# Cibiv/NextGenMap

Measured on AMD Instinct MI355X. Metric: mapped reads/sec + SW Gcells/sec, 150bp vs GRCh38, at 1/2/4/8 MI355X, higher is better.
Workload: dtype int32

## Files before the change

### include/ngm_pipeline.h

```cpp
#ifndef NGM_PIPELINE_H
#define NGM_PIPELINE_H

#include <stddef.h>
#include <stdint.h>

#ifdef __cplusplus
extern "C" {
#endif

typedef struct ngm_ref ngm_ref;
typedef struct ngm_mapper ngm_mapper;

typedef struct ngm_ref_params {
	int kmer;
	int kmer_skip;
	int bin_size;
} ngm_ref_params;

const char *ngm_pipeline_last_error(void);

ngm_ref *ngm_ref_create(int device, const ngm_ref_params *p, int n_contigs, const char *const *names,
		const uint8_t *const *seqs, const uint64_t *lens);
ngm_ref *ngm_ref_create_from_fasta(int device, const ngm_ref_params *p, const char *path);
ngm_ref *ngm_ref_create_from_cache(int device, const ngm_ref_params *params, const char *fasta_path);
// ... 127 lines not shown
int ngm_mapper_set_reference_cs_batch(ngm_mapper *m, int reads);

int ngm_mapper_path_counters(ngm_mapper *m, uint64_t out[8]);

int ngm_mapper_order_table_reads(ngm_mapper *m, uint64_t *out);

int ngm_debug_pair_walk(uint32_t cnt_a, int len_a, uint32_t cnt_b, int len_b, const uint32_t *loc, const uint32_t *sv, const float *score, const uint32_t *rank,
		float cutoff, int min_insert, int max_insert, uint32_t *out_a, uint32_t *out_b, int *mq_a, int *mq_b, uint64_t cap, float *combo_score, int *combo_dist, int *combo_a, int *combo_b,
		uint64_t *n_combo);

int ngm_debug_pair_eval(uint64_t n, const float *pair_score, const int *dist, const int *ia, const int *ib, int avg, int out_all[6], int out_kept[6]);

int ngm_debug_select_top1(int device, int n_reads, const uint32_t *base, const uint32_t *count, uint64_t n_cand, const float *scores, const uint32_t *loc,
		const uint32_t *strand_votes, uint32_t *winner, int32_t *mapq, int32_t *n_best, float *best_score);

int ngm_mapper_heavy_counters(ngm_mapper *m, uint64_t out[4]);

int ngm_mapper_cs_counters(ngm_mapper *m, uint64_t out[3]);

typedef struct ngm_stats_comm ngm_stats_comm;
int ngm_stats_unique_id(char hex[257]);
ngm_stats_comm *ngm_stats_comm_create(int device, int rank, int world, const char *hex);
int ngm_stats_allreduce(ngm_stats_comm *c, int64_t v[8]);
void ngm_stats_comm_destroy(ngm_stats_comm *c);
int ngm_mapper_last_pair_stats(ngm_mapper *m, uint64_t out[3]);

int ngm_mapper_last_kernel_ms(ngm_mapper *m, float ms[8]);
float ngm_mapper_last_order_replay_ms(ngm_mapper *m);

int ngm_mapper_set_argos(ngm_mapper *m, float min_score);
// ... 12 lines not shown
```

### nextgenmap_amd/csrc/cigar_device.h

```cpp
#pragma once

#include <hip/hip_runtime.h>
#include <stdint.h>

#include "sw_device.h"

namespace ngm {

struct CigarDevOut {
	uint32_t cig_off, md_off;
	uint16_t cig_len, md_len;
	int32_t position_offset, qstart, qend, nm;
	float identity, score_token;
	int32_t flags;
};

__device__ __forceinline__ uint32_t packed_class(const uint32_t *base, int m_base, int j) {
	const uint32_t w = base[(size_t) (m_base + (j >> 3)) * kSlots];
	const int b = j & 7;
	return (b < 4) ? (w >> (8 * b)) & 15u : (w >> (8 * (b - 4) + 4)) & 15u;
}
__device__ __forceinline__ char class_to_char(uint32_t c) {
	switch (c) { case 0: return 'A'; case 1: return 'C'; case 2: return 'G'; case 3: return 'T'; case 4: return 'x'; case 5: return 'N'; default: return 0; }
}
// ... 134 lines not shown
	__syncthreads();
	const unsigned long long base = s_base;
	if (!live) return;
	if (need) {
		if (base + total > capacity) o.flags &= ~1;
		else {
			const unsigned long long off = base + before;
			o.cig_off = (uint32_t) off; o.md_off = (uint32_t) off + o.cig_len;
			for (int t = 0; t < co; ++t) bytes[off + t] = cg[t];
			for (int t = 0; t < mo; ++t) bytes[off + co + t] = mdp[t];
		}
	}
	out[j] = o;
}

}
```

### nextgenmap_amd/csrc/engine_internal.h

```cpp
#pragma once

#include <algorithm>

#include <hip/hip_runtime.h>

#include <cstdint>
#include <string>

#include "../../include/ngm_hip.h"
#include "sw_device.h"
#include "affine_device.h"
#include "jit.h"

namespace ngm {
template <typename T>
struct DevBuf {
	T *p = nullptr;
	size_t cap = 0;
	int reserve(size_t n) {
		if (n <= cap) return 0;
		if (p) (void) hipFree(p);
		p = nullptr;
		cap = 0;
		const size_t want = n + std::min<size_t>(n / 8, ((size_t) 64 << 20) / sizeof(T));
		if (hipMalloc(&p, want * sizeof(T)) == hipSuccess) { cap = want; return 0; }
		if (hipMalloc(&p, n * sizeof(T)) != hipSuccess) return -1;
// ... 35 lines not shown
	ngm::DevBuf<uint32_t> packed;
	ngm::DevBuf<uint16_t> lens, blk_rows;
	ngm::DevBuf<uint8_t> d_ref, d_qry, d_pair_dir;
	const uint8_t *pair_dir = nullptr;
	ngm::DevBuf<float> d_scores;
	ngm::DevBuf<uint32_t> dirs;
	ngm::DevBuf<int32_t> d_records;
	ngm::DevBuf<uint16_t> d_runs;
	ngm::PinnedBuf<uint8_t> h_ref, h_qry;
	ngm::PinnedBuf<float> h_scores;
	ngm::PinnedBuf<int32_t> h_records;
	ngm::PinnedBuf<uint16_t> h_runs;
	bool profiling = false;
	hipEvent_t ev[4] = {nullptr, nullptr, nullptr, nullptr};
	bool ev_valid[3] = {false, false, false};
	std::string error;
};

namespace ngm {
int engine_reserve(ngm_hip_ctx *ctx, int n);
int engine_score_packed(ngm_hip_ctx *ctx, int mode, int n, float *d_scores, hipStream_t st);
int engine_align_packed(ngm_hip_ctx *ctx, int mode, int n, int32_t *d_records, uint16_t *d_runs, int run_stride, hipStream_t st);
}
```

### nextgenmap_amd/csrc/gather_device.h

```cpp
#pragma once

#include <hip/hip_runtime.h>
#include <stdint.h>

#include "sw_device.h"

namespace ngm {

struct WindowGeom {
	uint64_t concat_len;
	int buffer_len;
	int half_corridor;
};

__device__ __forceinline__ uint32_t window_class(const uint32_t *__restrict__ genome, const WindowGeom &G, uint64_t offset, int j) {
	uint64_t len = (uint64_t) G.buffer_len - 2;
	if (offset >= G.concat_len) return 5u;
	uint64_t end = 0;
	if (offset + len > G.concat_len) { end = offset + len - G.concat_len; len -= end; }
	const uint64_t emitted = ((offset & 1) ? 1 : 0) + 2 * ((len + 1) / 2);
	const uint64_t jj = (uint64_t) j;
	if (jj < emitted) {
		if ((len & 1) && jj == emitted - 1) return 4u;
		const uint64_t pos = offset + jj;
// ... 206 lines not shown
		if (small) { const uint32_t at = bs + (uint32_t) __popcll(ms & below); list_small[at] = (uint32_t) pi; info[pi] = -2 - (int32_t) at; }
		if (large) { const uint32_t at = bl + (uint32_t) __popcll(ml & below); list_large[at] = (uint32_t) pi; info[pi] = -2 - (int32_t) (at + (1u << 30)); }
		if (choice) return;
	}
	if (!live) return;
	if (ca != 1u || cb != 1u) { info[pi] = -1; return; }
	const uint32_t ba = cand_base[ra], bb = cand_base[rb];
	const uint64_t l1 = pair_loc[ba], l2 = pair_loc[bb];
	const int cur = (int) ((l2 > l1) ? l2 - l1 + (uint64_t) read_len[rb] : l1 - l2 + (uint64_t) read_len[ra]);
	const float ps = scores[ba] + scores[bb];
	const bool found = cur > min_d && cur < max_d && ps > 0.0f;
	if (found) { mapq[ra] = 60; mapq[rb] = 60; n_best[ra] = 0; n_best[rb] = 0; }
	info[pi] = found ? ((cur << 1) | 1) : 0;
}

__global__ void expand_pairs_kernel(int n_reads, const uint32_t *__restrict__ cand_base, const uint32_t *__restrict__ cand_count,
		uint32_t *__restrict__ pair_read) {
	const int r = blockIdx.x;
	const uint32_t b = cand_base[r], n = cand_count[r];
	for (uint32_t j = threadIdx.x; j < n; j += blockDim.x) pair_read[b + j] = (uint32_t) r;
}

__global__ void collect_winners_kernel(int n_reads, const uint32_t *__restrict__ winner, const uint32_t *__restrict__ pair_loc,
		const uint32_t *__restrict__ pair_sv, const uint32_t *__restrict__ slot_of_read, uint32_t *__restrict__ a_read,
		uint32_t *__restrict__ a_loc, uint32_t *__restrict__ a_sv) {
	const int r = blockIdx.x * blockDim.x + threadIdx.x;
	if (r >= n_reads) return;
	const uint32_t w = winner[r];
	if (w == 0xFFFFFFFFu) return;
	const uint32_t s = slot_of_read[r];
	a_read[s] = (uint32_t) r;
	a_loc[s] = pair_loc[w];
	a_sv[s] = pair_sv[w];
}

// ... 14 lines not shown
```

### nextgenmap_amd/csrc/mapper.cpp

```cpp
#define NGM_SAM_KERNELS
#include "mapper_internal.h"
#include <rocprim/rocprim.hpp>
#include "align_device.h"
#include "gather_device.h"

using ngm::DevGuard;
using ngm::GpuStage;
using ngm::run_cs;
using ngm::cs_host_arrays;
using ngm::candidate_order;
using ngm::candidate_order_wait;

namespace ngm {
StageLock g_stage_lock[16][2];
std::atomic<long long> g_stage_hold_us[3], g_stage_wait_us[3];
}
using ngm::g_stage_hold_us;
using ngm::g_stage_wait_us;

namespace {

int upload_reads(ngm_mapper *m, int n, const char *reads) {
	const size_t bytes = (size_t) n * m->prm.qry_max_len;
	if (m->d_reads.reserve(bytes)) { ngm::pipeline_set_error("out of device memory (reads)"); return -12; }
// ... 24 lines not shown
		char ch;
		if (jj < emitted) ch = ((len & 1) && jj == emitted - 1) ? 'x' : class_char(r->host_cls[offset + jj]);
		else if (jj < emitted + end) ch = 'x';
		else ch = 0;
		out[j] = ch;
	}
}

}

namespace ngm {
int score_candidates(ngm_mapper *m, int n, uint64_t np, int alt_dir) {
	const ngm_ref *r = m->ref;
	ngm_hip_ctx *eng = m->eng;
	const int q = m->prm.qry_max_len, c = m->prm.corridor;
	hipLaunchKernelGGL(ngm::expand_pairs_kernel, dim3(n), dim3(64), 0, m->st, n, m->d_cand_base.p, m->d_cand_count.p, m->d_pair_read.p);
	const int nb = (int) ((np + ngm::kSlots - 1) / ngm::kSlots);
	ngm::WindowGeom Gs{r->n_bases - 1, ((q + c) | 1) + 1, c >> 1};
	hipLaunchKernelGGL(ngm::gather_pairs_kernel, dim3(nb), dim3(256), 0, m->st, m->d_reads.p, m->d_read_len.p, q, r->d_genome, Gs,
			m->d_pair_read.p, m->d_out_loc.p, m->d_out_sv.p, (int) np, eng->RW, eng->FW, eng->packed.p, eng->lens.p, eng->blk_rows.p, alt_dir);
	MAP_HIP_TRY(hipGetLastError());
	MAP_HIP_TRY(hipEventRecord(m->ev[2], m->st));
	if (int rc = ngm::engine_score_packed(eng, m->prm.mode, (int) np, m->d_scores.p, m->st)) { ngm::pipeline_set_error("%s", ngm_hip_last_error(eng)); return rc; }
	MAP_HIP_TRY(hipEventRecord(m->ev[3], m->st));
	return 0;
}
}

extern "C" {

int ngm_ref_decode(const ngm_ref *r, uint64_t offset, int buffer_len, char *out) {
// ... 955 lines not shown
		if (m->d_a_read.reserve(na) || m->d_a_loc.reserve(na) || m->d_a_sv.reserve(na) || m->d_records.reserve((size_t) na * 8) ||
				m->d_runs.reserve((size_t) na * rs)) { ngm::pipeline_set_error("out of device memory (align stage)"); return -12; }
		if (int rc = ngm::engine_reserve(eng, na)) { ngm::pipeline_set_error("%s", ngm_hip_last_error(eng)); return rc; }
		MAP_HIP_TRY(hipMemcpyAsync(m->d_a_read.p, a_read.data(), (size_t) na * 4, hipMemcpyHostToDevice, m->st));
		MAP_HIP_TRY(hipMemcpyAsync(m->d_a_loc.p, a_loc.data(), (size_t) na * 4, hipMemcpyHostToDevice, m->st));
		MAP_HIP_TRY(hipMemcpyAsync(m->d_a_sv.p, a_sv.data(), (size_t) na * 4, hipMemcpyHostToDevice, m->st));
		MAP_HIP_TRY(hipStreamSynchronize(m->st));
		stage_align.acquire();
		MAP_HIP_TRY(hipEventRecord(m->ev[5], m->st));
		ngm::WindowGeom Ga{r->n_bases - 1, align_buf_len, c >> 1};
		hipLaunchKernelGGL(ngm::gather_pairs_kernel, dim3((na + ngm::kSlots - 1) / ngm::kSlots), dim3(256), 0, m->st, m->d_reads.p, m->d_read_len.p, q,
				r->d_genome, Ga, m->d_a_read.p, m->d_a_loc.p, m->d_a_sv.p, na, eng->RW, eng->FW, eng->packed.p, eng->lens.p, eng->blk_rows.p, alt_dir);
		MAP_HIP_TRY(hipGetLastError());
		MAP_HIP_TRY(hipEventRecord(m->ev[6], m->st));
		const bool was_prof = eng->profiling;
		eng->profiling = true;
		if (int rc = ngm::engine_align_packed(eng, mode, na, m->d_records.p, m->d_runs.p, rs, m->st)) { eng->profiling = was_prof; ngm::pipeline_set_error("%s", ngm_hip_last_error(eng)); return rc; }
		eng->profiling = was_prof;
		MAP_HIP_TRY(hipEventRecord(m->ev[7], m->st));
		if (m->d_runs_c.reserve((size_t) na * rs)) { ngm::pipeline_set_error("out of device memory (runs)"); return -12; }
		MAP_HIP_TRY(hipMemsetAsync(m->d_total.p, 0, 8, m->st));
		hipLaunchKernelGGL(ngm::compact_runs_kernel, dim3((na + 255) / 256), dim3(256), 0, m->st, na, m->d_records.p, m->d_runs.p, rs,
				m->d_runs_c.p, m->d_total.p);
		MAP_HIP_TRY(hipGetLastError());
		unsigned long long n_runs_total = 0, n_str_total = 0;
		if (!dev_strings) { MAP_HIP_TRY(hipEventRecord(m->ev[8], m->st)); }
		if (dev_strings) {
			const unsigned long long scap = (unsigned long long) na * 96ull + 4096ull;
			if (m->d_cigout.reserve(na) || m->d_str.reserve(scap) || m->p_cigout.reserve(na)) { ngm::pipeline_set_error("out of memory (CIGAR strings)"); return -12; }
			MAP_HIP_TRY(hipMemsetAsync(m->d_total.p + 8, 0, 8, m->st));
			const bool affine = m->prm.personality == NGM_PERSONALITY_AFFINE;
			if (affine) hipLaunchKernelGGL(ngm::cigar_strings_kernel<true>, dim3((na + 255) / 256), dim3(256), 0, m->st, na, m->d_records.p, m->d_runs_c.p, eng->packed.p, eng->RW, eng->FW,
					m->d_read_len.p, m->d_a_read.p, m->prm.variant == NGM_VARIANT_OCL_CPU ? 1 : 0, m->prm.hard_clip, m->prm.silent_clip, m->d_cigout.p, m->d_str.p, scap,
					(unsigned long long *) (m->d_total.p + 8), 0);
			else hipLaunchKernelGGL(ngm::cigar_strings_kernel<false>, dim3((na + 255) / 256), dim3(256), 0, m->st, na, m->d_records.p, m->d_runs_c.p, eng->packed.p, eng->RW, eng->FW,
					m->d_read_len.p, m->d_a_read.p, m->prm.variant == NGM_VARIANT_OCL_CPU ? 1 : 0, m->prm.hard_clip, m->prm.silent_clip, m->d_cigout.p, m->d_str.p, scap,
					(unsigned long long *) (m->d_total.p + 8), alt_cigar);
			MAP_HIP_TRY(hipGetLastError());
			MAP_HIP_TRY(hipEventRecord(m->ev[8], m->st));
			MAP_HIP_TRY(hipMemcpyAsync(m->p_cigout.p, m->d_cigout.p, (size_t) na * sizeof(ngm::CigarDevOut), hipMemcpyDeviceToHost, m->st));
			MAP_HIP_TRY(hipMemcpyAsync(&n_str_total, m->d_total.p + 8, 8, hipMemcpyDeviceToHost, m->st));
		}
		MAP_HIP_TRY(hipMemcpyAsync(h_rec, m->d_records.p, (size_t) na * 8 * 4, hipMemcpyDeviceToHost, m->st));
		MAP_HIP_TRY(hipMemcpyAsync(&n_runs_total, m->d_total.p, 8, hipMemcpyDeviceToHost, m->st));
		stage_align.done_after(m->ev[8]);
		MAP_HIP_TRY(hipStreamSynchronize(m->st));
		if (m->p_runs.reserve(n_runs_total + 1)) { ngm::pipeline_set_error("out of pinned host memory"); return -12; }
		h_runs = m->p_runs.p;
		MAP_HIP_TRY(hipMemcpy(h_runs, m->d_runs_c.p, n_runs_total * 2, hipMemcpyDeviceToHost));
		if (dev_strings) {
			n_str_total = std::min<unsigned long long>(n_str_total, (unsigned long long) na * 96ull + 4096ull);
			str_base = n_str_total;
			if (m->p_str.reserve(n_str_total + 1)) { ngm::pipeline_set_error("out of pinned host memory"); return -12; }
			if (n_str_total && !sam) MAP_HIP_TRY(hipMemcpy(m->p_str.p, m->d_str.p, n_str_total, hipMemcpyDeviceToHost));
		}
	}
	stage_align.done();

	lap(3);
	ngm::SamRef *sam_refs = sam ? m->p_sam_refs.p : nullptr;
	std::mutex extra_mu;
	std::vector<char> extra;
	parallel_for(n, [&](int lo, int hi) {
		for (int i = lo; i < hi; ++i) for (int t = 0; t < topn; ++t) {
			const size_t o = (size_t) i * topn + t;
			ngm_hit &h = hits[o];
			memset(&h, 0, sizeof(h));
			h.n_candidates = (int) m->h_count[i];
			h.max_votes = m->h_maxv[i];
// ... 298 lines not shown
		MAP_HIP_TRY(hipMemcpy(d_sc.p, scores, (size_t) n_cand * 4, hipMemcpyHostToDevice));
		MAP_HIP_TRY(hipMemcpy(d_loc.p, loc, (size_t) n_cand * 4, hipMemcpyHostToDevice));
		MAP_HIP_TRY(hipMemcpy(d_sv.p, strand_votes, (size_t) n_cand * 4, hipMemcpyHostToDevice));
	}
	hipLaunchKernelGGL(ngm::select_top1_kernel, dim3((n_reads + 255) / 256), dim3(256), 0, 0, n_reads, d_base.p, d_count.p, d_sc.p, d_loc.p, d_sv.p, d_win.p, d_mq.p, d_nb.p, d_best.p);
	MAP_HIP_TRY(hipGetLastError());
	MAP_HIP_TRY(hipDeviceSynchronize());
	MAP_HIP_TRY(hipMemcpy(winner, d_win.p, (size_t) n_reads * 4, hipMemcpyDeviceToHost));
	MAP_HIP_TRY(hipMemcpy(mapq, d_mq.p, (size_t) n_reads * 4, hipMemcpyDeviceToHost));
	MAP_HIP_TRY(hipMemcpy(n_best, d_nb.p, (size_t) n_reads * 4, hipMemcpyDeviceToHost));
	MAP_HIP_TRY(hipMemcpy(best_score, d_best.p, (size_t) n_reads * 4, hipMemcpyDeviceToHost));
	d_base.release(); d_count.release(); d_loc.release(); d_sv.release(); d_win.release(); d_mq.release(); d_nb.release(); d_sc.release(); d_best.release();
	return 0;
}

int ngm_mapper_heavy_counters(ngm_mapper *m, uint64_t out[4]) {
	if (!m || !out) return -22;
	out[0] = m->st_heavy_second; out[1] = m->st_heavy_restart; out[2] = m->st_heavy_sent_on; out[3] = m->st_pool_regrown;
	return 0;
}

int ngm_mapper_order_table_reads(ngm_mapper *m, uint64_t *out) {
	if (!m || !out) return -22;
	*out = m->st_order_table;
	return 0;
}

int ngm_mapper_cs_counters(ngm_mapper *m, uint64_t out[3]) {
	if (!m) return -22;
	out[0] = m->cs_kmers; out[1] = m->cs_hits; out[2] = m->n_cand;
// ... 19 lines not shown
```

### nextgenmap_amd/csrc/ngm_hip.cpp

```cpp
#include "../../include/ngm_hip.h"

#include <hip/hip_runtime.h>

#include <algorithm>

#include <cstdarg>
#include <cstdio>
#include <cstdlib>
#include <cstring>
#include <mutex>
#include <string>
#include <vector>

#define NGM_ENGINE_KERNELS
#include "engine_internal.h"
#include "align_device.h"
#include "affine_device.h"
#include "cigar_md.h"
#include "jit.h"

namespace {

thread_local std::string g_last_error;

// ... 139 lines not shown
	const bool endfree = (mode & NGM_MODE_ALIGN_MASK) == NGM_MODE_END_TO_END;
	if (!force32 && (long) ctx->q * std::max(ctx->K.tM, ctx->K.alt ? std::max(ctx->K.tMA, ctx->K.tXA) : 0) < 30000 && (long) ctx->q * ctx->K.tZ < 14000) {
		if (const void *pk = find_pk_score_kernel(ctx->c, endfree)) {
			KernelRef kp; kp.aot = pk;
			HIP_TRY(ctx, launch_kernel(kp, dim3((nb + 7) / 8), dim3(256), st, (const uint32_t *) ctx->packed.p, (const uint16_t *) ctx->lens.p,
					(const uint16_t *) ctx->blk_rows.p, d_scores, n, nb, ctx->RW, ctx->K));
			return 0;
		}
	}
	const KernelRef k = find_kernel(ctx, endfree ? 1 : 0);
	HIP_TRY(ctx, launch_kernel(k, dim3((nb + 3) / 4), dim3(256), st, (const uint32_t *) ctx->packed.p, (const uint16_t *) ctx->lens.p,
			(const uint16_t *) ctx->blk_rows.p, d_scores, n, nb, ctx->RW, ctx->K));
	return 0;
}

int engine_align_packed(ngm_hip_ctx *ctx, int mode, int n, int32_t *d_records, uint16_t *d_runs, int run_stride, hipStream_t st) {
	const int am = mode & NGM_MODE_ALIGN_MASK;
	const int nb = n_blocks_of(n);
	if (ctx->prm.personality == NGM_PERSONALITY_AFFINE) {
		const int CP = ctx->c + 1, ADW = ngm::aff_dir_words(CP);
		if (ctx->dirs.reserve((size_t) nb * ctx->q * ADW * ngm::kSlots)) { set_error(ctx, "out of device memory for the trace matrix"); return -12; }
		static const bool force32 = getenv("NGM_HIP_ALIGN_32BIT") != nullptr;
		const void *pk = nullptr;
		if (!force32 && am != NGM_MODE_END_TO_END && ctx->KA.open < 0 && ctx->KA.ext < 0 && (long) ctx->q * ctx->KA.tM < 30000 &&
				ctx->prm.gap_read_penalty + (long) ctx->q * (ctx->prm.gap_extend_penalty + ctx->KA.tZ) < 19000) {
			const bool plain_key = (long) ctx->q * ctx->prm.match_bonus < 2048 && ctx->c + 1 <= 32;
			if (plain_key) pk = find_pk_affine_align_kernel(ctx->c, false);
			else if (ctx->KA.tZ > 0 && ctx->KA.tM > 0 && ctx->KA.tM + 1 <= 63) pk = find_pk_affine_align_kernel(ctx->c, true);
		}
		if (pk) {
			KernelRef kp; kp.aot = pk;
			HIP_TRY(ctx, launch_kernel(kp, dim3((nb + 7) / 8), dim3(256), st, (const uint32_t *) ctx->packed.p, (const uint16_t *) ctx->lens.p,
					(const uint16_t *) ctx->blk_rows.p, ctx->dirs.p, d_records, n, nb, ctx->RW, ctx->q, ctx->KA));
		} else {
			const KernelRef ka = find_kernel(ctx, 6 + (am == NGM_MODE_END_TO_END ? 1 : 0));
			HIP_TRY(ctx, launch_kernel(ka, dim3((nb + 3) / 4), dim3(256), st, (const uint32_t *) ctx->packed.p, (const uint16_t *) ctx->lens.p,
					(const uint16_t *) ctx->blk_rows.p, (float *) nullptr, ctx->dirs.p, d_records, n, nb, ctx->RW, ctx->q, ctx->KA));
		}
		if (ctx->profiling) HIP_TRY(ctx, hipEventRecord(ctx->ev[2], st));
		hipLaunchKernelGGL(ngm::affine_traceback_kernel, dim3((n + 255) / 256), dim3(256), 0, st, ctx->dirs.p, d_records, d_runs, n,
				ctx->q, CP, run_stride, (const uint32_t *) ctx->packed.p, ctx->RW, ctx->FW, pk ? 1 : 0);
		HIP_TRY(ctx, hipGetLastError());
		return 0;
	}
	const int DW = ngm::dir_words(ctx->c);
	if (ctx->dirs.reserve((size_t) nb * ctx->q * DW * ngm::kSlots)) { set_error(ctx, "out of device memory for the direction matrix"); return -12; }
	static const bool force32 = getenv("NGM_HIP_ALIGN_32BIT") != nullptr;
	const void *pk = nullptr;
	const int max_gain = std::max(ctx->K.tM, ctx->K.alt ? std::max(ctx->K.tMA, ctx->K.tXA) : 0);
	if (!force32 && am != NGM_MODE_END_TO_END && (long) ctx->q * max_gain < 30000 && (long) ctx->q * ctx->K.tZ < 14000 && ctx->K.gl < 0 && ctx->K.gap_read < 0) {
		const bool plain_key = (long) ctx->q * (max_gain - ctx->K.tZ) < 2048 && ctx->c <= 32;
		if (plain_key) pk = find_pk_align_kernel(ctx->c, false);
		else if (ctx->K.tZ > 0 && max_gain + 1 <= 63) pk = find_pk_align_kernel(ctx->c, true);
	}
	if (pk) {
		KernelRef kp; kp.aot = pk;
		HIP_TRY(ctx, launch_kernel(kp, dim3((nb + 7) / 8), dim3(256), st, (const uint32_t *) ctx->packed.p, (const uint16_t *) ctx->lens.p,
				(const uint16_t *) ctx->blk_rows.p, ctx->dirs.p, d_records, n, nb, ctx->RW, ctx->q, ctx->K));
	} else {
// ... 246 lines not shown
	cp.variant = ctx->prm.variant;
	cp.hard_clip = ctx->prm.hard_clip;
	cp.silent_clip = ctx->prm.silent_clip;
	cp.alt = ctx->prm.alt_cigar;
	if (ctx->prm.personality == NGM_PERSONALITY_AFFINE) {
		for (int i = 0; i < n; ++i)
			ngm::build_cigar_affine(ctx->h_records.p + (size_t) i * 8, ctx->h_runs.p + (size_t) i * rs, ref[i], qry[i], ctx->q, &out[i]);
		return n;
	}
	for (int i = 0; i < n; ++i) {
		ngm::build_cigar_md(cp, ctx->h_records.p + (size_t) i * 8, ctx->h_runs.p + (size_t) i * rs, ref[i], qry[i], &out[i], (cp.alt && dir && dir[i]) ? 1 : 0);
	}
	return n;
}

}
```

### nextgenmap_amd/engine.py

```python
import ctypes as C
import os

import numpy as np

MODE_LOCAL = 0
MODE_END_TO_END = 1
VARIANT_OCL_GPU = 0
VARIANT_OCL_CPU = 1
PERSONALITY_LINEAR = 0
PERSONALITY_AFFINE = 1
ABI_VERSION = 3

_HERE = os.path.dirname(os.path.abspath(__file__))


class NgmHipError(RuntimeError):
    pass


class Params(C.Structure):
    _fields_ = [("abi_version", C.c_int), ("qry_max_len", C.c_int), ("corridor", C.c_int),
                ("match_bonus", C.c_int), ("mismatch_penalty", C.c_int), ("gap_read_penalty", C.c_int),
                ("gap_ref_penalty", C.c_int), ("variant", C.c_int), ("hard_clip", C.c_int),
                ("silent_clip", C.c_int), ("max_batch", C.c_int), ("personality", C.c_int),
# ... 28 lines not shown
    lib.ngm_hip_create.argtypes = [C.c_int, C.POINTER(Params)]
    lib.ngm_hip_destroy.argtypes = [C.c_void_p]
    lib.ngm_hip_last_error.restype = C.c_char_p
    lib.ngm_hip_last_error.argtypes = [C.c_void_p]
    lib.ngm_hip_device_count.restype = C.c_int
    lib.ngm_hip_score_batch_size.argtypes = [C.c_void_p]
    lib.ngm_hip_align_batch_size.argtypes = [C.c_void_p]
    lib.ngm_hip_batch_score.argtypes = [C.c_void_p, C.c_int, C.c_int, C.c_void_p, C.c_void_p, C.c_void_p, C.c_void_p]
    lib.ngm_hip_batch_align.argtypes = [C.c_void_p, C.c_int, C.c_int, C.c_void_p, C.c_void_p, C.c_void_p, C.c_void_p]
    lib.ngm_hip_score_device.argtypes = [C.c_void_p, C.c_int, C.c_int, C.c_void_p, C.c_void_p, C.c_void_p, C.c_void_p]
    lib.ngm_hip_align_run_stride.argtypes = [C.c_void_p]
    lib.ngm_hip_align_device.argtypes = [C.c_void_p, C.c_int, C.c_int, C.c_void_p, C.c_void_p, C.c_void_p, C.c_void_p,
                                         C.c_int, C.c_void_p]
    lib.ngm_hip_last_kernel_ms.argtypes = [C.c_void_p, C.POINTER(C.c_float)]
    lib.ngm_hip_set_profiling.argtypes = [C.c_void_p, C.c_int]
    _lib = lib
    return lib


def _ptr(x):
    if x is None:
        return None
    if hasattr(x, "data_ptr"):
        return x.data_ptr()
    return int(x)


class Engine:

    def __init__(self, qry_max_len, corridor, match=10, mismatch=15, gap_read=20, gap_ref=20, device=0,
# ... 35 lines not shown
        qry = np.ascontiguousarray(qry, dtype=np.uint8)
        n = qry.shape[0]
        assert qry.shape[1] >= self.q and ref.shape[1] >= self.q + self.c and ref.shape[0] == n
        rp = (C.c_void_p * n)(*[ref.ctypes.data + i * ref.strides[0] for i in range(n)])
        qp = (C.c_void_p * n)(*[qry.ctypes.data + i * qry.strides[0] for i in range(n)])
        return n, ref, qry, rp, qp

    def BatchScore(self, mode, ref, qry, dirs=None):
        n, ref, qry, rp, qp = self._ptr_lists(ref, qry)
        out = np.full(n, -1.0, dtype=np.float32)
        d = None if dirs is None else np.ascontiguousarray(dirs, dtype=np.uint8)
        r = self._check(self.lib.ngm_hip_batch_score(self.h, mode, n, rp, qp, out.ctypes.data, None if d is None else d.ctypes.data), n)
        assert r == n
        return out

    def BatchAlign(self, mode, ref, qry, dirs=None):
        n, ref, qry, rp, qp = self._ptr_lists(ref, qry)
        stride = 4 * max(1, self.q)
        cig = np.zeros((n, stride), dtype=np.uint8)
        md = np.zeros((n, stride), dtype=np.uint8)
        cig[:, :3] = ord("!")
        md[:, :3] = ord("!")
        outs = (AlignOut * n)()
        for i in range(n):
            outs[i].cigar = cig.ctypes.data + i * stride
            outs[i].md = md.ctypes.data + i * stride
        d = None if dirs is None else np.ascontiguousarray(dirs, dtype=np.uint8)
        r = self._check(self.lib.ngm_hip_batch_align(self.h, mode, n, rp, qp, outs, None if d is None else d.ctypes.data), n)
        assert r == n
        res = []
        for i in range(n):
            o = outs[i]
            res.append(dict(cigar=bytes(cig[i]).split(b"\0", 1)[0], md=bytes(md[i]).split(b"\0", 1)[0],
                            position_offset=o.position_offset, qstart=o.qstart, qend=o.qend,
                            score_token=o.score_token, identity=o.identity, nm=o.nm))
        return res

    def set_profiling(self, on):
        self.lib.ngm_hip_set_profiling(self.h, 1 if on else 0)

    def score_device(self, mode, n, d_ref, d_qry, d_scores, stream=None):
        return self._check(self.lib.ngm_hip_score_device(self.h, mode, n, _ptr(d_ref), _ptr(d_qry), _ptr(d_scores),
                                                          _ptr(stream)), n)
# ... 13 lines not shown
```

Measured before the change: 53.12 million.

## Fuse affine traceback and CIGAR string emission into one finishing kernel

Adds an affine_finish_kernel that walks the traceback directly from the direction matrix, counts matches and mismatches, and writes CIGAR strings into a device buffer. This skips the separate traceback, run compaction, run download and cigar_strings kernel on the affine top-1 path. Reads whose strings overflow fall back to the old traceback path. It also rewrites expand_pairs_kernel to use one thread per read, with wave-cooperative handling of reads that have many candidates, instead of one block per read. In exchange the finish path has more complex per-thread control flow and adds one extra host sync.

Result: faster. 57.62 million (median of 6 runs) (+8.5%).

```diff
diff --git a/include/ngm_pipeline.h b/include/ngm_pipeline.h
--- a/include/ngm_pipeline.h
+++ b/include/ngm_pipeline.h
@@ -165,6 +165,11 @@
 int ngm_debug_select_top1(int device, int n_reads, const uint32_t *base, const uint32_t *count, uint64_t n_cand, const float *scores, const uint32_t *loc,
 		const uint32_t *strand_votes, uint32_t *winner, int32_t *mapq, int32_t *n_best, float *best_score);
 
+int ngm_debug_align_finish(void *engine , int mode, int n, const char *const *ref, const char *const *qry, void *out ,
+		uint64_t *n_fallback);
+
+int ngm_debug_expand_pairs(int device, int n_reads, const uint32_t *base, const uint32_t *count, uint64_t n_cand, uint32_t *out);
+
 int ngm_mapper_heavy_counters(ngm_mapper *m, uint64_t out[4]);
 
 int ngm_mapper_cs_counters(ngm_mapper *m, uint64_t out[3]);
diff --git a/nextgenmap_amd/csrc/cigar_device.h b/nextgenmap_amd/csrc/cigar_device.h
--- a/nextgenmap_amd/csrc/cigar_device.h
+++ b/nextgenmap_amd/csrc/cigar_device.h
@@ -4,6 +4,7 @@
 #include <stdint.h>
 
 #include "sw_device.h"
+#include "affine_device.h"
 
 namespace ngm {
 
@@ -172,4 +173,178 @@
 	out[j] = o;
 }
 
-}
+constexpr int kFinishRows = 8;
+
+__device__ __forceinline__ uint32_t finish_sel8(uint32_t w0, uint32_t w1, uint32_t w2, uint32_t w3, uint32_t w4, uint32_t w5, uint32_t w6, uint32_t w7, int k) {
+	const uint32_t a0 = (k & 1) ? w1 : w0, a1 = (k & 1) ? w3 : w2, a2 = (k & 1) ? w5 : w4, a3 = (k & 1) ? w7 : w6;
+	const uint32_t b0 = (k & 2) ? a1 : a0, b1 = (k & 2) ? a3 : a2;
+	return (k & 4) ? b1 : b0;
+}
+
+template <bool NIBBLES>
+__global__ __launch_bounds__(256) void affine_finish_kernel(int n, const uint32_t *__restrict__ dirs, const int32_t *__restrict__ records,
+		const uint32_t *__restrict__ packed, const uint16_t *__restrict__ lens, int q, int CP, int RW, int FW, CigarDevOut *__restrict__ out,
+		char *__restrict__ bytes, unsigned long long capacity, unsigned long long *__restrict__ counters) {
+	__shared__ char s_rows[256 * kCigarRow];
+	__shared__ uint32_t s_wave[4];
+	__shared__ unsigned long long s_base;
+	const int j = blockIdx.x * blockDim.x + threadIdx.x;
+	const bool live = j < n;
+	const int lane = threadIdx.x & 63, wv = threadIdx.x >> 6;
+	constexpr int lim = kCigarRow - 16;
+	constexpr int WS = NIBBLES ? 3 : 2;
+	const int DW = NIBBLES ? aff_nib_words(CP) : aff_dir_words(CP);
+	char *row = s_rows + (size_t) threadIdx.x * kCigarRow;
+	int pos = kCigarRow;
+	auto put_back = [&](int num, char tag) {
+		row[--pos] = tag;
+		unsigned u = (unsigned) num;
+		do { row[--pos] = (char) ('0' + u % 10u); u /= 10u; } while (u);
+	};
+	bool fits = true;
+	int h = 0, v = 0, flags = 0, len_v = 0;
+	if (live) {
+		const int32_t *rec = records + (size_t) j * 8;
+		flags = rec[3]; h = rec[6]; v = rec[7];
+		len_v = (int) lens[j];
+	}
+	const int qend = len_v - v;
+	if (live && qend > 0) put_back(qend, 'S');
+	const int trail = kCigarRow - pos;
+	const uint32_t *dp = dirs + (size_t) (j >> 6) * q * DW * kSlots + lane;
+	const uint32_t *pk = packed + (size_t) (j >> 6) * (RW + FW) * kSlots + lane;
+	int cur = -1, curlen = 0, total = 0, n_match = 0, n_mis = 0;
+	bool done = !live, first = true, in_v = false, in_h = false;
+	auto flush = [&]() {
+		if (cur < 0) return;
+		if (kCigarRow - pos - trail > lim) { fits = false; done = true; return; }
+		put_back(curlen, cur == 1 ? 'M' : cur == 2 ? 'I' : 'D');
+		total += cur == 1 ? curlen : 1;
+	};
+	auto emit = [&](int op) {
+		if (op == cur) { ++curlen; return; }
+		flush();
+		cur = op; curlen = 1;
+	};
+	int gtop = (v - 1) >> 3;
+#pragma unroll
+	for (int s = 1; s < 64; s <<= 1) gtop = max(gtop, __shfl_xor(gtop, s));
+	for (int g = gtop; g >= 0; --g) {
+		const int r0 = g * kFinishRows;
+		const bool act = !done && v - 1 >= r0;
+		const int d0 = h - v;
+		const int wi = min(max(d0 >> WS, 0), DW - 1);
+		const int f0 = min(max((r0 + d0) >> 3, 0), FW - 1);
+		uint32_t W[kFinishRows];
+#pragma unroll
+		for (int k = 0; k < kFinishRows; ++k) W[k] = (act && r0 + k <= v - 1) ? dp[((size_t) (r0 + k) * DW + wi) * kSlots] : 0u;
+		const uint32_t rdw = act ? pk[(size_t) g * kSlots] : 0u;
+		const uint32_t fw0 = act ? pk[(size_t) (RW + f0) * kSlots] : 0u;
+		const uint32_t fw1 = (act && f0 + 1 < FW) ? pk[(size_t) (RW + f0 + 1) * kSlots] : 0u;
+		if (act && (!first || (NIBBLES && flags == 0)) && !in_v && !in_h) {
+			const int kc = v - 1 - r0;
+			if (d0 >= 0 && d0 < CP && (d0 >> WS) == wi && ((r0 + d0) >> 3) == f0 && f0 + 1 < FW) {
+				const int sh = NIBBLES ? 4 * (d0 & 7) : 8 * (d0 & 3);
+				uint32_t m = 0;
+#pragma unroll
+				for (int k = 0; k < kFinishRows; ++k) m |= (NIBBLES ? (uint32_t) (((W[k] >> sh) & 0xCu) == 4u) : ((W[k] >> sh) & 1u)) << k;
+				const uint32_t stop = ~m & ((2u << kc) - 1u);
+				const int lo = stop ? 32 - __clz((int) stop) : 0;
+				const int run = kc + 1 - lo;
+				if (run > 0) {
+					auto spread = [](uint32_t x) -> unsigned long long { return (unsigned long long) (x & 0x0F0F0F0Fu) | ((unsigned long long) ((x >> 4) & 0x0F0F0F0Fu) << 32); };
+					const unsigned long long ones = 0x0101010101010101ull, RB = spread(rdw), A = spread(fw0), B = spread(fw1);
+					const int o = (r0 + d0) & 7;
+					const unsigned long long WB = o ? (A >> (8 * o)) | (B << (64 - 8 * o)) : A;
+					const unsigned long long differ = (((RB ^ WB) + 0x0F0F0F0F0F0F0F0Full) >> 4) & ones;
+					const unsigned long long odd = (RB >> 2) & (~RB | (RB >> 1)) & ones;
+					const unsigned long long upto = kc == 7 ? ~0ull : (1ull << (8 * (kc + 1))) - 1ull;
+					const int mis = __popcll((differ | odd) & upto & ~((1ull << (8 * lo)) - 1ull));
+					n_mis += mis; n_match += run - mis;
+					if (cur != 1) { flush(); cur = 1; curlen = 0; }
+					curlen += run; h -= run; v -= run;
+					first = false;
+				}
+			}
+		}
+		while (!done && v - 1 >= r0) {
+			const int d = h - v;
+			uint32_t tv = 0u;
+			if (h > 0 && d >= 0 && d < CP) {
+				const int w = d >> WS;
+				const uint32_t word = (w == wi) ? finish_sel8(W[0], W[1], W[2], W[3], W[4], W[5], W[6], W[7], v - 1 - r0) : dp[((size_t) (v - 1) * DW + w) * kSlots];
+				tv = NIBBLES ? aff_trace_from_nibble((word >> (4 * (d & 7))) & 15u, d, CP) : (word >> (8 * (d & 3))) & 0xFFu;
+			}
+			if (first) {
+				first = false;
+				if (flags & 1) tv = (tv & ~(uint32_t) kTDiag) | (uint32_t) kTMaxV;
+				else if (flags & 2) tv = (tv & ~(uint32_t) kTDiag) | (uint32_t) kTMaxH;
+				if (tv & kTMaxV) tv &= (uint32_t) (kTVert | kTVertOpen | kTMaxV);
+				else if (tv & kTMaxH) tv &= (uint32_t) (kTHori | kTHoriOpen | kTMaxH);
+			}
+			if (!in_v && !in_h) {
+				if (h <= 0 || tv == 0u) { done = true; break; }
+				if (tv & kTDiag) {
+					emit(1);
+					const int jr = (v - 1) & 7, jf = (h - 1) & 7, fi = (h - 1) >> 3;
+					const uint32_t fx = (fi == f0) ? fw0 : (fi == f0 + 1) ? fw1 : pk[(size_t) (RW + fi) * kSlots];
+					const uint32_t rc = (rdw >> (4 * ((jr & 3) * 2 + (jr >> 2)))) & 15u, fc = (fx >> (4 * ((jf & 3) * 2 + (jf >> 2)))) & 15u;
+					if (rc == fc && rc <= 5u && rc != 4u) ++n_match; else ++n_mis;
+					--h; --v;
+					continue;
+				}
+				if ((tv & kTMaxV) && (tv & kTVert)) in_v = true;
+				else if ((tv & kTMaxV) && (tv & kTVertOpen)) { emit(2); --v; continue; }
+				else if ((tv & kTMaxH) && (tv & kTHori)) in_h = true;
+				else if ((tv & kTMaxH) && (tv & kTHoriOpen)) { emit(3); --h; continue; }
+				else { done = true; break; }
+			}
+			if (in_v) { in_v = (!(tv & kTVertOpen) || (tv & kTVert)) && v != 1; emit(2); --v; }
+			else { in_h = (!(tv & kTHoriOpen) || (tv & kTHori)) && h != 1; emit(3); --h; }
+		}
+	}
+	int co = 0;
+	if (live) {
+		if (fits) flush();
+		int lead = 0;
+		if (v > 0) { lead = 2; for (int t = v; t >= 10; t /= 10) ++lead; }
+		if (kCigarRow - pos - trail + lead > lim) fits = false;
+		if (fits && v > 0) put_back(v, 'S');
+		co = kCigarRow - pos;
+	}
+	constexpr int mo = 3;
+	const uint32_t need = (live && fits) ? (uint32_t) (co + mo) : 0u;
+	uint32_t incl = need;
+#pragma unroll
+	for (int d = 1; d < 64; d <<= 1) { const uint32_t t = __shfl_up(incl, d); if (lane >= d) incl += t; }
+	if (lane == 63) s_wave[wv] = incl;
+	__syncthreads();
+	uint32_t before = incl - need, total_b = 0;
+#pragma unroll
+	for (int w2 = 0; w2 < 4; ++w2) { if (w2 < wv) before += s_wave[w2]; total_b += s_wave[w2]; }
+	if (threadIdx.x == 0) s_base = total_b ? atomicAdd(&counters[0], (unsigned long long) total_b) : 0ull;
+	__syncthreads();
+	const unsigned long long base = s_base;
+	if (!live) return;
+	uint32_t cig_off = 0;
+	if (need) {
+		if (base + total_b > capacity) fits = false;
+		else {
+			const unsigned long long off = base + before;
+			cig_off = (uint32_t) off;
+			const char *cg = row + pos;
+			for (int t = 0; t < co; ++t) bytes[off + t] = cg[t];
+			for (int t = 0; t < mo; ++t) bytes[off + co + t] = '!';
+		}
+	}
+	if (!fits) atomicAdd(&counters[1], 1ull);
+	CigarDevOut *o = out + j;
+	o->cig_off = cig_off; o->md_off = fits ? cig_off + (uint32_t) co : 0u;
+	o->cig_len = (uint16_t) co; o->md_len = (uint16_t) mo;
+	o->position_offset = h; o->qstart = v; o->qend = qend; o->nm = n_mis;
+	o->identity = (float) n_match * 1.0f / (float) total;
+	o->score_token = 0.f;
+	o->flags = (fits ? 1 : 0) | 2;
+}
+
+}
diff --git a/nextgenmap_amd/csrc/engine_internal.h b/nextgenmap_amd/csrc/engine_internal.h
--- a/nextgenmap_amd/csrc/engine_internal.h
+++ b/nextgenmap_amd/csrc/engine_internal.h
@@ -10,6 +10,7 @@
 #include "../../include/ngm_hip.h"
 #include "sw_device.h"
 #include "affine_device.h"
+#include "cigar_device.h"
 #include "jit.h"
 
 namespace ngm {
@@ -75,11 +76,19 @@
 	bool profiling = false;
 	hipEvent_t ev[4] = {nullptr, nullptr, nullptr, nullptr};
 	bool ev_valid[3] = {false, false, false};
+	bool trace_nibbles = false;
 	std::string error;
 };
 
 namespace ngm {
 int engine_reserve(ngm_hip_ctx *ctx, int n);
 int engine_score_packed(ngm_hip_ctx *ctx, int mode, int n, float *d_scores, hipStream_t st);
-int engine_align_packed(ngm_hip_ctx *ctx, int mode, int n, int32_t *d_records, uint16_t *d_runs, int run_stride, hipStream_t st);
+struct AlignFinish {
+	CigarDevOut *out;
+	char *bytes;
+	unsigned long long capacity;
+	unsigned long long *counters;
+};
+int engine_align_packed(ngm_hip_ctx *ctx, int mode, int n, int32_t *d_records, uint16_t *d_runs, int run_stride, hipStream_t st, const AlignFinish *fin = nullptr);
+int engine_affine_traceback_packed(ngm_hip_ctx *ctx, int n, int32_t *d_records, uint16_t *d_runs, int run_stride, hipStream_t st);
 }
diff --git a/nextgenmap_amd/csrc/gather_device.h b/nextgenmap_amd/csrc/gather_device.h
--- a/nextgenmap_amd/csrc/gather_device.h
+++ b/nextgenmap_amd/csrc/gather_device.h
@@ -244,11 +244,25 @@
 	info[pi] = found ? ((cur << 1) | 1) : 0;
 }
 
-__global__ void expand_pairs_kernel(int n_reads, const uint32_t *__restrict__ cand_base, const uint32_t *__restrict__ cand_count,
+__global__ __launch_bounds__(256) void expand_pairs_kernel(int n_reads, const uint32_t *__restrict__ cand_base, const uint32_t *__restrict__ cand_count,
 		uint32_t *__restrict__ pair_read) {
-	const int r = blockIdx.x;
-	const uint32_t b = cand_base[r], n = cand_count[r];
-	for (uint32_t j = threadIdx.x; j < n; j += blockDim.x) pair_read[b + j] = (uint32_t) r;
+	__shared__ uint32_t s_big[256], s_nbig;
+	const int tid = threadIdx.x, lane = tid & 63, wv = tid >> 6;
+	if (tid == 0) s_nbig = 0;
+	__syncthreads();
+	const int r = blockIdx.x * 256 + tid;
+	if (r < n_reads) {
+		const uint32_t b = cand_base[r], n = cand_count[r];
+		if (n <= kSelectSmall) { for (uint32_t j = 0; j < n; ++j) pair_read[b + j] = (uint32_t) r; }
+		else s_big[atomicAdd(&s_nbig, 1u)] = (uint32_t) tid;
+	}
+	__syncthreads();
+	const uint32_t nbig = s_nbig;
+	for (uint32_t i = (uint32_t) wv; i < nbig; i += 4u) {
+		const int rr = blockIdx.x * 256 + (int) s_big[i];
+		const uint32_t b = cand_base[rr], n = cand_count[rr];
+		for (uint32_t j = (uint32_t) lane; j < n; j += 64u) pair_read[b + j] = (uint32_t) rr;
+	}
 }
 
 __global__ void collect_winners_kernel(int n_reads, const uint32_t *__restrict__ winner, const uint32_t *__restrict__ pair_loc,
diff --git a/nextgenmap_amd/csrc/mapper.cpp b/nextgenmap_amd/csrc/mapper.cpp
--- a/nextgenmap_amd/csrc/mapper.cpp
+++ b/nextgenmap_amd/csrc/mapper.cpp
@@ -62,7 +62,7 @@
 	const ngm_ref *r = m->ref;
 	ngm_hip_ctx *eng = m->eng;
 	const int q = m->prm.qry_max_len, c = m->prm.corridor;
-	hipLaunchKernelGGL(ngm::expand_pairs_kernel, dim3(n), dim3(64), 0, m->st, n, m->d_cand_base.p, m->d_cand_count.p, m->d_pair_read.p);
+	hipLaunchKernelGGL(ngm::expand_pairs_kernel, dim3((n + 255) / 256), dim3(256), 0, m->st, n, m->d_cand_base.p, m->d_cand_count.p, m->d_pair_read.p);
 	const int nb = (int) ((np + ngm::kSlots - 1) / ngm::kSlots);
 	ngm::WindowGeom Gs{r->n_bases - 1, ((q + c) | 1) + 1, c >> 1};
 	hipLaunchKernelGGL(ngm::gather_pairs_kernel, dim3(nb), dim3(256), 0, m->st, m->d_reads.p, m->d_read_len.p, q, r->d_genome, Gs,
@@ -1048,6 +1048,44 @@
 		MAP_HIP_TRY(hipGetLastError());
 		MAP_HIP_TRY(hipEventRecord(m->ev[6], m->st));
 		const bool was_prof = eng->profiling;
+		const bool affine = m->prm.personality == NGM_PERSONALITY_AFFINE;
+		static const bool tail_split = getenv("NGM_HIP_ALIGN_TAIL_SPLIT") != nullptr;
+		const bool finish = affine && dev_strings && topn == 1 && !tail_split;
+		const unsigned long long scap = (unsigned long long) na * 96ull + 4096ull;
+		unsigned long long n_runs_total = 0, n_str_total = 0;
+		if (dev_strings && (m->d_cigout.reserve(na) || m->d_str.reserve(scap) || m->p_cigout.reserve(na))) { ngm::pipeline_set_error("out of memory (CIGAR strings)"); return -12; }
+		if (finish) {
+			unsigned long long ctr[2] = {0, 0};
+			MAP_HIP_TRY(hipMemsetAsync(m->d_total.p + 8, 0, 16, m->st));
+			const ngm::AlignFinish fin{m->d_cigout.p, m->d_str.p, scap, m->d_total.p + 8};
+			eng->profiling = true;
+			if (int rc = ngm::engine_align_packed(eng, mode, na, m->d_records.p, m->d_runs.p, rs, m->st, &fin)) { eng->profiling = was_prof; ngm::pipeline_set_error("%s", ngm_hip_last_error(eng)); return rc; }
+			eng->profiling = was_prof;
+			MAP_HIP_TRY(hipEventRecord(m->ev[7], m->st));
+			MAP_HIP_TRY(hipEventRecord(m->ev[8], m->st));
+			MAP_HIP_TRY(hipMemcpyAsync(m->p_cigout.p, m->d_cigout.p, (size_t) na * sizeof(ngm::CigarDevOut), hipMemcpyDeviceToHost, m->st));
+			MAP_HIP_TRY(hipMemcpyAsync(ctr, m->d_total.p + 8, 16, hipMemcpyDeviceToHost, m->st));
+			stage_align.done_after(m->ev[8]);
+			MAP_HIP_TRY(hipStreamSynchronize(m->st));
+			n_str_total = std::min<unsigned long long>(ctr[0], scap);
+			str_base = n_str_total;
+			if (m->p_str.reserve(n_str_total + 1)) { ngm::pipeline_set_error("out of pinned host memory"); return -12; }
+			if (n_str_total && !sam) MAP_HIP_TRY(hipMemcpy(m->p_str.p, m->d_str.p, n_str_total, hipMemcpyDeviceToHost));
+			if (ctr[1]) {
+				if (m->d_runs_c.reserve((size_t) na * rs)) { ngm::pipeline_set_error("out of device memory (runs)"); return -12; }
+				MAP_HIP_TRY(hipMemsetAsync(m->d_total.p, 0, 8, m->st));
+				if (int rc = ngm::engine_affine_traceback_packed(eng, na, m->d_records.p, m->d_runs.p, rs, m->st)) { ngm::pipeline_set_error("%s", ngm_hip_last_error(eng)); return rc; }
+				hipLaunchKernelGGL(ngm::compact_runs_kernel, dim3((na + 255) / 256), dim3(256), 0, m->st, na, m->d_records.p, m->d_runs.p, rs,
+						m->d_runs_c.p, m->d_total.p);
+				MAP_HIP_TRY(hipGetLastError());
+				MAP_HIP_TRY(hipMemcpyAsync(h_rec, m->d_records.p, (size_t) na * 8 * 4, hipMemcpyDeviceToHost, m->st));
+				MAP_HIP_TRY(hipMemcpyAsync(&n_runs_total, m->d_total.p, 8, hipMemcpyDeviceToHost, m->st));
+				MAP_HIP_TRY(hipStreamSynchronize(m->st));
+				if (m->p_runs.reserve(n_runs_total + 1)) { ngm::pipeline_set_error("out of pinned host memory"); return -12; }
+				h_runs = m->p_runs.p;
+				MAP_HIP_TRY(hipMemcpy(h_runs, m->d_runs_c.p, n_runs_total * 2, hipMemcpyDeviceToHost));
+			}
+		} else {
 		eng->profiling = true;
 		if (int rc = ngm::engine_align_packed(eng, mode, na, m->d_records.p, m->d_runs.p, rs, m->st)) { eng->profiling = was_prof; ngm::pipeline_set_error("%s", ngm_hip_last_error(eng)); return rc; }
 		eng->profiling = was_prof;
@@ -1057,13 +1095,9 @@
 		hipLaunchKernelGGL(ngm::compact_runs_kernel, dim3((na + 255) / 256), dim3(256), 0, m->st, na, m->d_records.p, m->d_runs.p, rs,
 				m->d_runs_c.p, m->d_total.p);
 		MAP_HIP_TRY(hipGetLastError());
-		unsigned long long n_runs_total = 0, n_str_total = 0;
 		if (!dev_strings) { MAP_HIP_TRY(hipEventRecord(m->ev[8], m->st)); }
 		if (dev_strings) {
-			const unsigned long long scap = (unsigned long long) na * 96ull + 4096ull;
-			if (m->d_cigout.reserve(na) || m->d_str.reserve(scap) || m->p_cigout.reserve(na)) { ngm::pipeline_set_error("out of memory (CIGAR strings)"); return -12; }
 			MAP_HIP_TRY(hipMemsetAsync(m->d_total.p + 8, 0, 8, m->st));
-			const bool affine = m->prm.personality == NGM_PERSONALITY_AFFINE;
 			if (affine) hipLaunchKernelGGL(ngm::cigar_strings_kernel<true>, dim3((na + 255) / 256), dim3(256), 0, m->st, na, m->d_records.p, m->d_runs_c.p, eng->packed.p, eng->RW, eng->FW,
 					m->d_read_len.p, m->d_a_read.p, m->prm.variant == NGM_VARIANT_OCL_CPU ? 1 : 0, m->prm.hard_clip, m->prm.silent_clip, m->d_cigout.p, m->d_str.p, scap,
 					(unsigned long long *) (m->d_total.p + 8), 0);
@@ -1083,10 +1117,11 @@
 		h_runs = m->p_runs.p;
 		MAP_HIP_TRY(hipMemcpy(h_runs, m->d_runs_c.p, n_runs_total * 2, hipMemcpyDeviceToHost));
 		if (dev_strings) {
-			n_str_total = std::min<unsigned long long>(n_str_total, (unsigned long long) na * 96ull + 4096ull);
+			n_str_total = std::min<unsigned long long>(n_str_total, scap);
 			str_base = n_str_total;
 			if (m->p_str.reserve(n_str_total + 1)) { ngm::pipeline_set_error("out of pinned host memory"); return -12; }
 			if (n_str_total && !sam) MAP_HIP_TRY(hipMemcpy(m->p_str.p, m->d_str.p, n_str_total, hipMemcpyDeviceToHost));
+		}
 		}
 	}
 	stage_align.done();
@@ -1415,6 +1450,26 @@
 	return 0;
 }
 
+int ngm_debug_expand_pairs(int device, int n_reads, const uint32_t *base, const uint32_t *count, uint64_t n_cand, uint32_t *out) {
+	if (n_reads <= 0 || !base || !count || (n_cand && !out)) return -22;
+	DevGuard g(device);
+	ngm::DevBuf<uint32_t> d_base, d_count, d_out;
+	auto run = [&]() -> int {
+		if (d_base.reserve(n_reads) || d_count.reserve(n_reads) || d_out.reserve((size_t) std::max<uint64_t>(n_cand, 1))) { ngm::pipeline_set_error("out of device memory (ngm_debug_expand_pairs)"); return -12; }
+		MAP_HIP_TRY(hipMemcpy(d_base.p, base, (size_t) n_reads * 4, hipMemcpyHostToDevice));
+		MAP_HIP_TRY(hipMemcpy(d_count.p, count, (size_t) n_reads * 4, hipMemcpyHostToDevice));
+		MAP_HIP_TRY(hipMemset(d_out.p, 0xFF, (size_t) std::max<uint64_t>(n_cand, 1) * 4));
+		hipLaunchKernelGGL(ngm::expand_pairs_kernel, dim3((n_reads + 255) / 256), dim3(256), 0, 0, n_reads, d_base.p, d_count.p, d_out.p);
+		MAP_HIP_TRY(hipGetLastError());
+		MAP_HIP_TRY(hipDeviceSynchronize());
+		if (n_cand) MAP_HIP_TRY(hipMemcpy(out, d_out.p, (size_t) n_cand * 4, hipMemcpyDeviceToHost));
+		return 0;
+	};
+	const int rc = run();
+	d_base.release(); d_count.release(); d_out.release();
+	return rc;
+}
+
 int ngm_mapper_heavy_counters(ngm_mapper *m, uint64_t out[4]) {
 	if (!m || !out) return -22;
 	out[0] = m->st_heavy_second; out[1] = m->st_heavy_restart; out[2] = m->st_heavy_sent_on; out[3] = m->st_pool_regrown;
diff --git a/nextgenmap_amd/csrc/ngm_hip.cpp b/nextgenmap_amd/csrc/ngm_hip.cpp
--- a/nextgenmap_amd/csrc/ngm_hip.cpp
+++ b/nextgenmap_amd/csrc/ngm_hip.cpp
@@ -1,4 +1,5 @@
 #include "../../include/ngm_hip.h"
+#include "../../include/ngm_pipeline.h"
 
 #include <hip/hip_runtime.h>
 
@@ -177,7 +178,14 @@
 	return 0;
 }
 
-int engine_align_packed(ngm_hip_ctx *ctx, int mode, int n, int32_t *d_records, uint16_t *d_runs, int run_stride, hipStream_t st) {
+int engine_affine_traceback_packed(ngm_hip_ctx *ctx, int n, int32_t *d_records, uint16_t *d_runs, int run_stride, hipStream_t st) {
+	hipLaunchKernelGGL(ngm::affine_traceback_kernel, dim3((n + 255) / 256), dim3(256), 0, st, ctx->dirs.p, d_records, d_runs, n,
+			ctx->q, ctx->c + 1, run_stride, (const uint32_t *) ctx->packed.p, ctx->RW, ctx->FW, ctx->trace_nibbles ? 1 : 0);
+	HIP_TRY(ctx, hipGetLastError());
+	return 0;
+}
+
+int engine_align_packed(ngm_hip_ctx *ctx, int mode, int n, int32_t *d_records, uint16_t *d_runs, int run_stride, hipStream_t st, const AlignFinish *fin) {
 	const int am = mode & NGM_MODE_ALIGN_MASK;
 	const int nb = n_blocks_of(n);
 	if (ctx->prm.personality == NGM_PERSONALITY_AFFINE) {
@@ -201,11 +209,16 @@
 					(const uint16_t *) ctx->blk_rows.p, (float *) nullptr, ctx->dirs.p, d_records, n, nb, ctx->RW, ctx->q, ctx->KA));
 		}
 		if (ctx->profiling) HIP_TRY(ctx, hipEventRecord(ctx->ev[2], st));
-		hipLaunchKernelGGL(ngm::affine_traceback_kernel, dim3((n + 255) / 256), dim3(256), 0, st, ctx->dirs.p, d_records, d_runs, n,
-				ctx->q, CP, run_stride, (const uint32_t *) ctx->packed.p, ctx->RW, ctx->FW, pk ? 1 : 0);
+		ctx->trace_nibbles = pk != nullptr;
+		if (!fin) return engine_affine_traceback_packed(ctx, n, d_records, d_runs, run_stride, st);
+		if (pk) hipLaunchKernelGGL(ngm::affine_finish_kernel<true>, dim3((n + 255) / 256), dim3(256), 0, st, n, (const uint32_t *) ctx->dirs.p, (const int32_t *) d_records,
+				(const uint32_t *) ctx->packed.p, (const uint16_t *) ctx->lens.p, ctx->q, CP, ctx->RW, ctx->FW, fin->out, fin->bytes, fin->capacity, fin->counters);
+		else hipLaunchKernelGGL(ngm::affine_finish_kernel<false>, dim3((n + 255) / 256), dim3(256), 0, st, n, (const uint32_t *) ctx->dirs.p, (const int32_t *) d_records,
+				(const uint32_t *) ctx->packed.p, (const uint16_t *) ctx->lens.p, ctx->q, CP, ctx->RW, ctx->FW, fin->out, fin->bytes, fin->capacity, fin->counters);
 		HIP_TRY(ctx, hipGetLastError());
 		return 0;
 	}
+	if (fin) { set_error(ctx, "the finishing kernel serves the affine personality only"); return -22; }
 	const int DW = ngm::dir_words(ctx->c);
 	if (ctx->dirs.reserve((size_t) nb * ctx->q * DW * ngm::kSlots)) { set_error(ctx, "out of device memory for the direction matrix"); return -12; }
 	static const bool force32 = getenv("NGM_HIP_ALIGN_32BIT") != nullptr;
@@ -482,4 +495,70 @@
 	return n;
 }
 
-}
+int ngm_debug_align_finish(void *engine, int mode, int n, const char *const *ref, const char *const *qry, void *out_records, uint64_t *n_fallback) {
+	ngm_hip_ctx *ctx = (ngm_hip_ctx *) engine;
+	ngm_hip_align_out *out = (ngm_hip_align_out *) out_records;
+	if (!ctx || !out || !n_fallback) return -22;
+	*n_fallback = 0;
+	if (n <= 0) return 0;
+	if (ctx->prm.personality != NGM_PERSONALITY_AFFINE) { set_error(ctx, "ngm_debug_align_finish: affine personality only"); return -22; }
+	const int am = mode & NGM_MODE_ALIGN_MASK;
+	if (am != NGM_MODE_LOCAL && am != NGM_MODE_END_TO_END) { set_error(ctx, "unsupported alignment mode %d", am); return -22; }
+	ScopedDevice sd(ctx->device);
+	const size_t rl = ctx->rl, q = ctx->q;
+	const int rs = ngm::run_stride(ctx->q, ctx->c);
+	if (ctx->h_ref.reserve((size_t) n * rl) || ctx->h_qry.reserve((size_t) n * q) || ctx->d_ref.reserve((size_t) n * rl) ||
+			ctx->d_qry.reserve((size_t) n * q) || ctx->d_records.reserve((size_t) n * 8) || ctx->d_runs.reserve((size_t) n * rs) ||
+			ctx->h_records.reserve((size_t) n * 8) || ctx->h_runs.reserve((size_t) n * rs)) {
+		set_error(ctx, "out of memory staging %d pairs", n);
+		return -12;
+	}
+	for (int i = 0; i < n; ++i) {
+		memcpy(ctx->h_ref.p + (size_t) i * rl, ref[i], rl);
+		memcpy(ctx->h_qry.p + (size_t) i * q, qry[i], q);
+	}
+	const unsigned long long scap = (unsigned long long) n * ngm::kCigarRow + 4096ull;
+	ngm::DevBuf<ngm::CigarDevOut> d_out;
+	ngm::DevBuf<char> d_str;
+	ngm::DevBuf<unsigned long long> d_ctr;
+	std::vector<ngm::CigarDevOut> h_out((size_t) n);
+	std::vector<char> h_str((size_t) scap);
+	unsigned long long ctr[2] = {0, 0};
+	auto run = [&]() -> int {
+		if (d_out.reserve(n) || d_str.reserve(scap) || d_ctr.reserve(2)) { set_error(ctx, "out of device memory (ngm_debug_align_finish)"); return -12; }
+		HIP_TRY(ctx, hipMemcpyAsync(ctx->d_ref.p, ctx->h_ref.p, (size_t) n * rl, hipMemcpyHostToDevice, ctx->stream));
+		HIP_TRY(ctx, hipMemcpyAsync(ctx->d_qry.p, ctx->h_qry.p, (size_t) n * q, hipMemcpyHostToDevice, ctx->stream));
+		HIP_TRY(ctx, hipMemsetAsync(d_ctr.p, 0, 16, ctx->stream));
+		if (int r = engine_reserve(ctx, n)) return r;
+		if (int r = launch_pack(ctx, n, ctx->d_ref.p, ctx->d_qry.p, ctx->stream)) return r;
+		const ngm::AlignFinish fin{d_out.p, d_str.p, scap, d_ctr.p};
+		if (int r = ngm::engine_align_packed(ctx, mode, n, ctx->d_records.p, ctx->d_runs.p, rs, ctx->stream, &fin)) return r;
+		HIP_TRY(ctx, hipMemcpyAsync(h_out.data(), d_out.p, (size_t) n * sizeof(ngm::CigarDevOut), hipMemcpyDeviceToHost, ctx->stream));
+		HIP_TRY(ctx, hipMemcpyAsync(ctr, d_ctr.p, 16, hipMemcpyDeviceToHost, ctx->stream));
+		HIP_TRY(ctx, hipStreamSynchronize(ctx->stream));
+		const unsigned long long used = std::min(ctr[0], scap);
+		if (used) HIP_TRY(ctx, hipMemcpy(h_str.data(), d_str.p, (size_t) used, hipMemcpyDeviceToHost));
+		if (ctr[1]) {
+			if (int r = ngm::engine_affine_traceback_packed(ctx, n, ctx->d_records.p, ctx->d_runs.p, rs, ctx->stream)) return r;
+			HIP_TRY(ctx, hipMemcpyAsync(ctx->h_records.p, ctx->d_records.p, sizeof(int32_t) * 8 * (size_t) n, hipMemcpyDeviceToHost, ctx->stream));
+			HIP_TRY(ctx, hipMemcpyAsync(ctx->h_runs.p, ctx->d_runs.p, sizeof(uint16_t) * (size_t) rs * n, hipMemcpyDeviceToHost, ctx->stream));
+			HIP_TRY(ctx, hipStreamSynchronize(ctx->stream));
+		}
+		return 0;
+	};
+	const int rc = run();
+	d_out.release(); d_str.release(); d_ctr.release();
+	if (rc) return rc;
+	*n_fallback = ctr[1];
+	for (int i = 0; i < n; ++i) {
+		const ngm::CigarDevOut &dv = h_out[(size_t) i];
+		if (!(dv.flags & 1)) { ngm::build_cigar_affine(ctx->h_records.p + (size_t) i * 8, ctx->h_runs.p + (size_t) i * rs, ref[i], qry[i], ctx->q, &out[i]); continue; }
+		memcpy(out[i].cigar, h_str.data() + dv.cig_off, dv.cig_len); out[i].cigar[dv.cig_len] = 0;
+		memcpy(out[i].md, h_str.data() + dv.md_off, dv.md_len); out[i].md[dv.md_len] = 0;
+		out[i].position_offset = dv.position_offset; out[i].qstart = dv.qstart; out[i].qend = dv.qend;
+		out[i].score_token = dv.score_token; out[i].identity = dv.identity; out[i].nm = dv.nm;
+	}
+	return n;
+}
+
+}
diff --git a/nextgenmap_amd/engine.py b/nextgenmap_amd/engine.py
--- a/nextgenmap_amd/engine.py
+++ b/nextgenmap_amd/engine.py
@@ -66,6 +66,7 @@
                                          C.c_int, C.c_void_p]
     lib.ngm_hip_last_kernel_ms.argtypes = [C.c_void_p, C.POINTER(C.c_float)]
     lib.ngm_hip_set_profiling.argtypes = [C.c_void_p, C.c_int]
+    lib.ngm_debug_align_finish.argtypes = [C.c_void_p, C.c_int, C.c_int, C.c_void_p, C.c_void_p, C.c_void_p, C.POINTER(C.c_uint64)]
     _lib = lib
     return lib
 
@@ -131,7 +132,7 @@
         assert r == n
         return out
 
-    def BatchAlign(self, mode, ref, qry, dirs=None):
+    def BatchAlign(self, mode, ref, qry, dirs=None, finish=False):
         n, ref, qry, rp, qp = self._ptr_lists(ref, qry)
         stride = 4 * max(1, self.q)
         cig = np.zeros((n, stride), dtype=np.uint8)
@@ -143,7 +144,12 @@
             outs[i].cigar = cig.ctypes.data + i * stride
             outs[i].md = md.ctypes.data + i * stride
         d = None if dirs is None else np.ascontiguousarray(dirs, dtype=np.uint8)
-        r = self._check(self.lib.ngm_hip_batch_align(self.h, mode, n, rp, qp, outs, None if d is None else d.ctypes.data), n)
+        if finish:
+            fb = C.c_uint64(0)
+            r = self._check(self.lib.ngm_debug_align_finish(self.h, mode, n, rp, qp, outs, C.byref(fb)), n)
+            self.last_fallback = int(fb.value)
+        else:
+            r = self._check(self.lib.ngm_hip_batch_align(self.h, mode, n, rp, qp, outs, None if d is None else d.ctypes.data), n)
         assert r == n
         res = []
         for i in range(n):
```
